# bharatlytics/faceRecognition_InfrenceEngine

Hardware: AMD Instinct MI355X
Metric: faces/sec end-to-end @1080p (higher is better)
Workload: dtype f16

## Files before the change

### facerecognition_infrenceengine_amd/csrc/ro_conv2.hip

```cpp
#include "detect_math.h"

namespace {

struct Rc2Args {
    const unsigned char* xs;
    const float* w;
    const float* bias; const float* slope;
    float* y;
    const int32_t* counts; int cap;
    int nslots, per_block;
    int32_t* zero;
};

template <int WIN, int HB, int WOUT, int HC, int G, int NCT, int NPH, int NBAND, int BROWS, int PR, int PO, int PROUNDS, int NBUFS, int DEPTH_>
struct Rc2Cfg {
    static constexpr int P = WIN + 2;
    static constexpr int NPX = G * HC * WOUT;
    static constexpr int NT = (NPX + 15) / 16;
    static constexpr int NTW = (NT + NPH - 1) / NPH;
    static constexpr int PLANE = G * HB * P * 64;
    static constexpr int NW = NCT * NPH;
    static constexpr int NPIECE = (2 * PLANE + 1023) / 1024;
    static constexpr int NPW = (NPIECE + NW - 1) / NW;
    static constexpr int COUT = NCT * 16;
    static constexpr int PC = COUT / PROUNDS;
    static constexpr int CS = PC + 4;
    static constexpr int POOL_BYTES = NPX * CS * 4;
    static constexpr int BUF = NPIECE * 1024 > POOL_BYTES ? NPIECE * 1024 : (POOL_BYTES + 1023) / 1024 * 1024;
    static constexpr int PRM_OFF = NBUFS * BUF;
    static constexpr int LDS_BYTES = PRM_OFF + 2 * COUT * 4;
    static constexpr int SLOT_BYTES = WIN * WIN * 128;
    static constexpr int KC = WOUT % 8, GK = (HC * WOUT) % 8;
    static constexpr int NTHR = NW * 64;
    static constexpr int NSTEP = 9 * NTW;
    static constexpr int DEPTH = DEPTH_;
    static constexpr int DMA_EVERY = (NSTEP * 5 / 8) / NPW > 0 ? (NSTEP * 5 / 8) / NPW : 1;
    static constexpr int Q4 = PC / 4;
    static_assert(NBUFS == 1 || NSTEP - 4 >= NPW, "every piece of the next item is issued inside the K loop");
    static_assert(NCT % PROUNDS == 0, "pool rounds");
    static_assert(2 * PLANE + 3 * P * 64 < 65536, "ds_read immediates");
    static_assert(2 * (PR - 1) + 2 < HC && 2 * (PO - 1) + 2 < WOUT + 0 * BROWS, "pool windows lie inside the band");
};

template <int WIN, int HB, int WOUT, int HC, int G, int NCT, int NPH, int NBAND, int BROWS, int PR, int PO, int PROUNDS, int NBUFS, int DEPTH_, int MINW>
__global__ __launch_bounds__(NCT * NPH * 64, MINW) void ro_conv2_split_kernel(Rc2Args a) {
#if defined(__HIP_DEVICE_COMPILE__)
    using C = Rc2Cfg<WIN, HB, WOUT, HC, G, NCT, NPH, NBAND, BROWS, PR, PO, PROUNDS, NBUFS, DEPTH_>;
    extern __shared__ __attribute__((aligned(16))) char lds2[];
    const int tid = threadIdx.x, lane = tid & 63, wave = tid >> 6;
    const int li = lane & 15, kq = lane >> 4;
    const int ct = wave % NCT, ph = wave / NCT;
    const int nitems = (a.nslots + G - 1) / G * NBAND;
    const int it_end = min(nitems, (int)(blockIdx.x + 1) * a.per_block);
    if (a.zero && blockIdx.x == 0 && tid == 0) *a.zero = 0;
    auto next_valid = [&](int it) {
        while (it < it_end) {
            const int s0 = it / NBAND * G;
            bool any = false;
            int last = s0;
#pragma unroll
            for (int g = 0; g < G; ++g) {
                const int sl = s0 + g;
                if (sl < a.nslots) {
                    const int f = sl / a.cap;
                    any = any || sl - f * a.cap < a.counts[f];
                    last = sl;
                }
            }
            if (any) return it;
            const int nxt = ((last / a.cap + 1) * a.cap) / G * NBAND;
            it = nxt > it ? nxt : it + 1;
        }
        return -1;
    };
    int cur = next_valid(blockIdx.x * a.per_block);
    if (cur < 0) return;

    half8 wh[9], wl[9];
    {
        const float* wrow = a.w + (size_t)(ct * 16 + li) * 9 * 32 + 8 * kq;
#pragma unroll
        for (int tap = 0; tap < 9; ++tap) {
            const float4v v0 = *reinterpret_cast<const float4v*>(wrow + tap * 32);
            const float4v v1 = *reinterpret_cast<const float4v*>(wrow + tap * 32 + 4);
#pragma unroll
            for (int j = 0; j < 8; ++j) {
                split_f16(j < 4 ? v0[j] : v1[j - 4], wh[tap], wl[tap], j);
            }
        }
    }
    const float4v bias_r = *reinterpret_cast<const float4v*>(a.bias + ct * 16 + 4 * kq);
    const float4v slope_r = *reinterpret_cast<const float4v*>(a.slope + ct * 16 + 4 * kq);
    bool mono = true;
    for (int c = 0; c < C::COUT; ++c) mono = mono && a.slope[c] >= 0.f;

    unsigned voff[C::NPW];
#pragma unroll
    for (int i = 0; i < C::NPW; ++i) {
        const int n = (wave + C::NW * i) * 64 + lane;
        unsigned o = 0x80000000u;
        if (n < 2 * C::PLANE / 16) {
            const int pl = n / (C::PLANE / 16), m = n - pl * (C::PLANE / 16);
            const int row = m >> 2, cp = m & 3;
            const int g = row / (HB * C::P), rr = row - g * (HB * C::P);
            const int Y = rr / C::P, X = rr - Y * C::P;
            if (X < WIN) {
                const int key = ((X + C::KC * Y + C::GK * g) >> 1) & 3;
                o = (unsigned)(g * C::SLOT_BYTES + (Y * WIN + X) * 128 + pl * 64 + ((cp ^ key) << 4));
            }
        }
        voff[i] = o;
    }
    auto item_rsrc = [&](int it) {
        const int sg = it / NBAND, band = it - sg * NBAND;
        const int s0 = sg * G;
        const unsigned char* base = a.xs + (size_t)s0 * C::SLOT_BYTES + (size_t)band * BROWS * WIN * 128;
        const int nsl = min(G, a.nslots - s0);
        const unsigned bytes = NBAND == 1 ? (unsigned)nsl * C::SLOT_BYTES : (unsigned)(HB * WIN * 128);
        return buffer_rsrc(base, bytes);
    };
    auto piece = [&](__amdgpu_buffer_rsrc_t rs, int buf, int i) {
        const int j = wave + C::NW * i;
        if (j < C::NPIECE)
            __builtin_amdgcn_raw_ptr_buffer_load_lds(rs, (lds_ptr_t)(lds2 + buf * C::BUF + j * 1024), 16, voff[i], 0, 0, 0);
    };
    const unsigned lbase = (unsigned)reinterpret_cast<uintptr_t>((lds_ptr_t)lds2);
    unsigned rt[C::NTW];
#pragma unroll
    for (int k = 0; k < C::NTW; ++k) {
        const int q = min((ph + k * NPH) * 16 + li, C::NPX - 1);
        const int g = q / (HC * WOUT), qq = q - g * (HC * WOUT);
        const int y = qq / WOUT, x = qq - y * WOUT;
        rt[k] = lbase + ((g * HB + y) * C::P + x) * 64;
    }

    float* prm = reinterpret_cast<float*>(lds2 + C::PRM_OFF);
    for (int c = tid; c < C::COUT; c += C::NTHR) { prm[c] = a.bias[c]; prm[C::COUT + c] = a.slope[c]; }
    if (NBUFS == 2) {
        const __amdgpu_buffer_rsrc_t rs0 = item_rsrc(cur);
#pragma unroll
        for (int i = 0; i < C::NPW; ++i) piece(rs0, 0, i);
    }
    int nxt = next_valid(cur + 1);
    for (int b = 0; cur >= 0; b ^= (NBUFS - 1)) {
        const int sg = cur / NBAND, band = cur - sg * NBAND;
        const int s0 = sg * G;
        unsigned smask = 0;
#pragma unroll
        for (int g = 0; g < G; ++g) {
            const int sl = s0 + g;
            if (sl < a.nslots) {
                const int f = sl / a.cap;
                if (sl - f * a.cap < a.counts[f]) smask |= 1u << g;
            }
        }
        if (NBUFS == 1) {
            __syncthreads();
            const __amdgpu_buffer_rsrc_t rs0 = item_rsrc(cur);
#pragma unroll
            for (int i = 0; i < C::NPW; ++i) piece(rs0, 0, i);
        }
        asm volatile("s_waitcnt vmcnt(0)" ::: "memory");
        __syncthreads();
        const __amdgpu_buffer_rsrc_t rsn = item_rsrc(nxt >= 0 ? nxt : cur);
        const int nn = nxt >= 0 ? next_valid(nxt + 1) : -1;

        float4v acc[C::NTW];
#pragma unroll
        for (int k = 0; k < C::NTW; ++k) acc[k] = float4v{0.f, 0.f, 0.f, 0.f};
        const unsigned boff = b ? (unsigned)C::BUF : 0u;
        unsigned xd[8];
#pragma unroll
        for (int d = 0; d < 8; ++d) xd[d] = boff + (unsigned)((kq ^ (((li + d) & 7) >> 1)) << 4);
        half8 fh[C::DEPTH + 1], fl[C::DEPTH + 1];
        auto rd = [&](auto S) {
            constexpr int s = decltype(S)::value;
            constexpr int tap = s / C::NTW, k = s - tap * C::NTW, kh = tap / 3, kw = tap - kh * 3;
            constexpr int imm = (kh * C::P + kw) * 64;
            unsigned ad;
            const unsigned r0 = rt[k], x0 = xd[(kw + C::KC * kh) & 7];
            half8& h = fh[s % (C::DEPTH + 1)];
            half8& l = fl[s % (C::DEPTH + 1)];
            asm volatile("v_add_u32 %2, %3, %4\n\tds_read_b128 %0, %2 offset:%5\n\tds_read_b128 %1, %2 offset:%6"
                         : "=&v"(h), "=&v"(l), "=&v"(ad)
                         : "v"(r0), "v"(x0), "n"(imm), "n"(imm + C::PLANE));
        };
        static_for<C::DEPTH>([&](auto S) { rd(S); });
        static_for<C::NSTEP>([&](auto S) {
            constexpr int s = decltype(S)::value;
            constexpr int tap = s / C::NTW, k = s - tap * C::NTW;
            if constexpr (s + C::DEPTH < C::NSTEP) rd(std::integral_constant<int, s + C::DEPTH>{});
            if constexpr (NBUFS == 2 && s >= 2 && (s - 2) % C::DMA_EVERY == 0 && (s - 2) / C::DMA_EVERY < C::NPW) {
                if (nxt >= 0) piece(rsn, b ^ 1, (s - 2) / C::DMA_EVERY);
            }
            constexpr int later = (C::NSTEP - 1 - s) < C::DEPTH ? (C::NSTEP - 1 - s) : C::DEPTH;
            half8& bh = fh[s % (C::DEPTH + 1)];
            half8& bl = fl[s % (C::DEPTH + 1)];
            asm volatile("s_waitcnt lgkmcnt(%2)" : "+v"(bh), "+v"(bl) : "n"(2 * later));
            acc[k] = __builtin_amdgcn_mfma_f32_16x16x32_f16(wh[tap], bh, acc[k], 0, 0, 0);
            acc[k] = __builtin_amdgcn_mfma_f32_16x16x32_f16(wl[tap], bh, acc[k], 0, 0, 0);
            acc[k] = __builtin_amdgcn_mfma_f32_16x16x32_f16(wh[tap], bl, acc[k], 0, 0, 0);
        });

        float* pt = reinterpret_cast<float*>(lds2 + b * C::BUF);
#pragma unroll
        for (int round = 0; round < PROUNDS; ++round) {
            __syncthreads();
            if (ct / (NCT / PROUNDS) == round) {
#pragma unroll
                for (int k = 0; k < C::NTW; ++k) {
                    const int q = (ph + k * NPH) * 16 + li;
                    if (q < C::NPX) {
                        float4v v = acc[k];
                        if (!mono) {
                            v += bias_r;
#pragma unroll
                            for (int e = 0; e < 4; ++e) v[e] = v[e] > 0.f ? v[e] : v[e] * slope_r[e];
                        }
                        *reinterpret_cast<float4v*>(pt + q * C::CS + (ct % (NCT / PROUNDS)) * 16 + 4 * kq) = v;
                    }
                }
            }
            __syncthreads();
            constexpr int Q4 = C::Q4;
            for (int e = tid; e < G * PR * PO * Q4; e += C::NTHR) {
                const int qd = e % Q4, pp = e / Q4;
                const int g = pp / (PR * PO), p2 = pp - g * (PR * PO);
                const int pr = p2 / PO, pc = p2 - pr * PO;
                const int slot = s0 + g;
                if (!((smask >> g) & 1)) continue;
                const float* src = pt + ((g * HC + 2 * pr) * WOUT + 2 * pc) * C::CS + qd * 4;
                float4v m = *reinterpret_cast<const float4v*>(src);
#pragma unroll
                for (int dy = 0; dy < 3; ++dy)
#pragma unroll
                    for (int dx = 0; dx < 3; ++dx) {
                        if (dy == 0 && dx == 0) continue;
                        const float4v v = *reinterpret_cast<const float4v*>(src + (dy * WOUT + dx) * C::CS);
#pragma unroll
                        for (int k = 0; k < 4; ++k) m[k] = fmaxf(m[k], v[k]);
                    }
                const int co = round * C::PC + qd * 4;
                if (mono) {
                    m += *reinterpret_cast<const float4v*>(prm + co);
                    const float4v sv = *reinterpret_cast<const float4v*>(prm + C::COUT + co);
#pragma unroll
                    for (int k = 0; k < 4; ++k) m[k] = m[k] > 0.f ? m[k] : m[k] * sv[k];
                }
                *reinterpret_cast<float4v*>(a.y + (((size_t)slot * PO + band * PR + pr) * PO + pc) * C::COUT + co) = m;
            }
        }
        cur = nxt; nxt = nn;
    }
#endif
}

template <int WIN, int HB, int WOUT, int HC, int G, int NCT, int NPH, int NBAND, int BROWS, int PR, int PO, int PROUNDS, int NBUFS, int DEPTH_, int MINW>
int launch_rc2(Rc2Args a, hipStream_t s) {
    using C = Rc2Cfg<WIN, HB, WOUT, HC, G, NCT, NPH, NBAND, BROWS, PR, PO, PROUNDS, NBUFS, DEPTH_>;
    auto kern = ro_conv2_split_kernel<WIN, HB, WOUT, HC, G, NCT, NPH, NBAND, BROWS, PR, PO, PROUNDS, NBUFS, DEPTH_, MINW>;
    const size_t lds = C::LDS_BYTES;
    if (lds > 64 * 1024) {
        static FrDevLatch latch;
        if (!fr_raise_lds(reinterpret_cast<const void*>(kern), lds, latch)) {
            fr_set_error("fr_ro_conv2_split: cannot raise dynamic LDS to %zu bytes", lds);
            return FR_E_LAUNCH;
        }
    }
    const int nitems = (a.nslots + G - 1) / G * NBAND;
    const int resident = 256 * (MINW * 4 / C::NW);
    int per = (nitems + 2 * resident - 1) / (2 * resident);
    if (per < 1) per = 1;
    a.per_block = per;
    kern<<<(nitems + per - 1) / per, C::NTHR, lds, s>>>(a);
    return FR_OK;
}

__global__ void ro_margin_list_kernel(const float* head, int nhead, const int32_t* counts, int nslots, int cap, float lthr,
                                      float margin, int32_t* list, int32_t* lcount, int lcap) {
    const int slot = blockIdx.x * 256 + threadIdx.x;
    if (slot >= nslots) return;
    const int f = slot / cap;
    if (slot - f * cap >= counts[f]) return;
    const float* h = head + (size_t)slot * nhead;
    const float d = h[1] - h[0];
    bool nonfinite = split_nonfinite(d);
    for (int i = 2; i < nhead; ++i) nonfinite = nonfinite || split_nonfinite(h[i]);
    if (nonfinite || fabsf(d - lthr) <= margin) {
        const int pos = atomicAdd(lcount, 1);
        if (pos < lcap) list[pos] = slot;
    }
}

__global__ void ro_scatter_rows_kernel(const float* src, const int32_t* list, const int32_t* lcount, int lcap, int ncols, float* dst) {
    const int n = min(*lcount, lcap);
    const int e = blockIdx.x * 256 + threadIdx.x;
    const int i = e / ncols, c = e - i * ncols;
    if (i < n) dst[(size_t)list[i] * ncols + c] = src[(size_t)i * ncols + c];
}

}

extern "C" int fr_ro_conv2_split(int net, const void* x_split, const float* w, const float* bias, const float* slope, float* y,
                                 int nslots, const int32_t* counts, int cap, int32_t* zero_word, fr_stream_t stream) {
    FR_REQUIRE(x_split && w && bias && slope && y && counts, "fr_ro_conv2_split: null pointer");
    FR_REQUIRE(nslots > 0 && cap > 0 && nslots % cap == 0, "fr_ro_conv2_split: nslots must be frames x cap");
    Rc2Args a{(const unsigned char*)x_split, w, bias, slope, y, counts, cap, nslots, 1, zero_word};
    hipStream_t s = fr_stream(stream);
    int rc;
    if (net == 0) rc = launch_rc2<11, 11, 9, 9, 3, 3, 4, 1, 0, 4, 4, 1, 2, 2, 3>(a, s);
    else if (net == 1) rc = launch_rc2<23, 13, 21, 11, 1, 4, 1, 2, 10, 5, 10, 1, 1, 3, 2>(a, s);
    else { FR_REQUIRE(false, "fr_ro_conv2_split: net must be 0 (R-Net) or 1 (O-Net)"); }
    if (rc != FR_OK) return rc;
    FR_CHECK_LAUNCH("ro_conv2_split_kernel");
    return FR_OK;
}

extern "C" int fr_ro_margin_list(const float* head, int nhead, const int32_t* counts, int nframes, int cap, float logit_thr,
                                 float margin, int32_t* list, int32_t* list_count, int list_cap, fr_stream_t stream) {
    FR_REQUIRE(head && counts && list && list_count, "fr_ro_margin_list: null pointer");
    FR_REQUIRE(nhead >= 2 && nframes > 0 && cap > 0 && list_cap > 0 && margin >= 0.f, "fr_ro_margin_list: bad argument");
    hipStream_t s = fr_stream(stream);
    const int nslots = nframes * cap;
    ro_margin_list_kernel<<<(nslots + 255) / 256, 256, 0, s>>>(head, nhead, counts, nslots, cap, logit_thr, margin, list, list_count, list_cap);
    FR_CHECK_LAUNCH("ro_margin_list_kernel");
    return FR_OK;
}

extern "C" int fr_ro_scatter_rows(const float* src, const int32_t* list, const int32_t* list_count, int list_cap, int ncols,
                                  float* dst, fr_stream_t stream) {
    FR_REQUIRE(src && list && list_count && dst && list_cap > 0 && ncols > 0, "fr_ro_scatter_rows: bad argument");
    ro_scatter_rows_kernel<<<(list_cap * ncols + 255) / 256, 256, 0, fr_stream(stream)>>>(src, list, list_count, list_cap, ncols, dst);
    FR_CHECK_LAUNCH("ro_scatter_rows_kernel");
    return FR_OK;
}
```

Baseline: 25360.

## Overlap R-Net conv2 max-pool of previous item with next item's MFMA loop

For the R-Net configuration, the conv2 kernel now writes each item's activations to a dedicated LDS tile. The 3x3 max-pool and store of that item is deferred into the next item's K loop, with groups of four waves taking turns at staggered steps, so pooling and global stores hide behind MFMA work. Slot-validity masks are now computed once in next_valid, which reads counts through scalar constant loads and is moved into the middle of the K loop. Max uses fmed3 against +inf. The extra LDS tile raises shared memory per block, which may cut occupancy, and the DMA issue schedule shifts later in the loop.

```diff
diff --git a/facerecognition_infrenceengine_amd/csrc/ro_conv2.hip b/facerecognition_infrenceengine_amd/csrc/ro_conv2.hip
--- a/facerecognition_infrenceengine_amd/csrc/ro_conv2.hip
+++ b/facerecognition_infrenceengine_amd/csrc/ro_conv2.hip
@@ -1,6 +1,17 @@
 #include "detect_math.h"
 
 namespace {
+
+__device__ __forceinline__ float opaque_inf() {
+    float r;
+    asm("v_mov_b32 %0, 0x7f800000" : "=v"(r));
+    return r;
+}
+__device__ __forceinline__ float vmax(float x, float y, float pinf) { return __builtin_amdgcn_fmed3f(x, y, pinf); }
+
+__device__ __forceinline__ int32_t ld_uniform(const int32_t* p, int i) {
+    return reinterpret_cast<const __attribute__((address_space(4))) int32_t*>(reinterpret_cast<uintptr_t>(p))[i];
+}
 
 struct Rc2Args {
     const unsigned char* xs;
@@ -12,7 +23,7 @@
     int32_t* zero;
 };
 
-template <int WIN, int HB, int WOUT, int HC, int G, int NCT, int NPH, int NBAND, int BROWS, int PR, int PO, int PROUNDS, int NBUFS, int DEPTH_>
+template <int WIN, int HB, int WOUT, int HC, int G, int NCT, int NPH, int NBAND, int BROWS, int PR, int PO, int PROUNDS, int NBUFS, int DEPTH_, bool OVL>
 struct Rc2Cfg {
     static constexpr int P = WIN + 2;
     static constexpr int NPX = G * HC * WOUT;
@@ -26,8 +37,11 @@
     static constexpr int PC = COUT / PROUNDS;
     static constexpr int CS = PC + 4;
     static constexpr int POOL_BYTES = NPX * CS * 4;
-    static constexpr int BUF = NPIECE * 1024 > POOL_BYTES ? NPIECE * 1024 : (POOL_BYTES + 1023) / 1024 * 1024;
-    static constexpr int PRM_OFF = NBUFS * BUF;
+    static constexpr int TCS = COUT + 4;
+    static constexpr int TILE_BYTES = NPX * TCS * 4;
+    static constexpr int BUF = OVL || NPIECE * 1024 > POOL_BYTES ? NPIECE * 1024 : (POOL_BYTES + 1023) / 1024 * 1024;
+    static constexpr int TILE_OFF = NBUFS * BUF;
+    static constexpr int PRM_OFF = TILE_OFF + (OVL ? TILE_BYTES : 0);
     static constexpr int LDS_BYTES = PRM_OFF + 2 * COUT * 4;
     static constexpr int SLOT_BYTES = WIN * WIN * 128;
     static constexpr int KC = WOUT % 8, GK = (HC * WOUT) % 8;
@@ -36,16 +50,21 @@
     static constexpr int DEPTH = DEPTH_;
     static constexpr int DMA_EVERY = (NSTEP * 5 / 8) / NPW > 0 ? (NSTEP * 5 / 8) / NPW : 1;
     static constexpr int Q4 = PC / 4;
+    static constexpr int PSLOTS = NW / 4;
+    static constexpr int PGAP = 2;
+    static constexpr int DMA0 = OVL ? 2 + (PSLOTS - 1) * PGAP : 2;
+    static_assert(!OVL || (NBUFS == 2 && PROUNDS == 1 && NW % 4 == 0), "overlapped pool");
+    static_assert(NBUFS == 1 || DMA0 + (NPW - 1) * DMA_EVERY <= NSTEP - 4, "the last piece is issued well inside the K loop");
     static_assert(NBUFS == 1 || NSTEP - 4 >= NPW, "every piece of the next item is issued inside the K loop");
     static_assert(NCT % PROUNDS == 0, "pool rounds");
     static_assert(2 * PLANE + 3 * P * 64 < 65536, "ds_read immediates");
     static_assert(2 * (PR - 1) + 2 < HC && 2 * (PO - 1) + 2 < WOUT + 0 * BROWS, "pool windows lie inside the band");
 };
 
-template <int WIN, int HB, int WOUT, int HC, int G, int NCT, int NPH, int NBAND, int BROWS, int PR, int PO, int PROUNDS, int NBUFS, int DEPTH_, int MINW>
+template <int WIN, int HB, int WOUT, int HC, int G, int NCT, int NPH, int NBAND, int BROWS, int PR, int PO, int PROUNDS, int NBUFS, int DEPTH_, int MINW, bool OVL>
 __global__ __launch_bounds__(NCT * NPH * 64, MINW) void ro_conv2_split_kernel(Rc2Args a) {
 #if defined(__HIP_DEVICE_COMPILE__)
-    using C = Rc2Cfg<WIN, HB, WOUT, HC, G, NCT, NPH, NBAND, BROWS, PR, PO, PROUNDS, NBUFS, DEPTH_>;
+    using C = Rc2Cfg<WIN, HB, WOUT, HC, G, NCT, NPH, NBAND, BROWS, PR, PO, PROUNDS, NBUFS, DEPTH_, OVL>;
     extern __shared__ __attribute__((aligned(16))) char lds2[];
     const int tid = threadIdx.x, lane = tid & 63, wave = tid >> 6;
     const int li = lane & 15, kq = lane >> 4;
@@ -53,27 +72,29 @@
     const int nitems = (a.nslots + G - 1) / G * NBAND;
     const int it_end = min(nitems, (int)(blockIdx.x + 1) * a.per_block);
     if (a.zero && blockIdx.x == 0 && tid == 0) *a.zero = 0;
-    auto next_valid = [&](int it) {
+    auto next_valid = [&](int it, unsigned& mask) {
         while (it < it_end) {
             const int s0 = it / NBAND * G;
-            bool any = false;
+            unsigned m = 0;
             int last = s0;
 #pragma unroll
             for (int g = 0; g < G; ++g) {
                 const int sl = s0 + g;
                 if (sl < a.nslots) {
                     const int f = sl / a.cap;
-                    any = any || sl - f * a.cap < a.counts[f];
+                    if (sl - f * a.cap < ld_uniform(a.counts, f)) m |= 1u << g;
                     last = sl;
                 }
             }
-            if (any) return it;
+            if (m) { mask = m; return it; }
             const int nxt = ((last / a.cap + 1) * a.cap) / G * NBAND;
             it = nxt > it ? nxt : it + 1;
         }
+        mask = 0;
         return -1;
     };
-    int cur = next_valid(blockIdx.x * a.per_block);
+    unsigned smask, nxt_mask;
+    int cur = next_valid(blockIdx.x * a.per_block, smask);
     if (cur < 0) return;
 
     half8 wh[9], wl[9];
@@ -134,6 +155,8 @@
         rt[k] = lbase + ((g * HB + y) * C::P + x) * 64;
     }
 
+    const float pinf = opaque_inf();
+
     float* prm = reinterpret_cast<float*>(lds2 + C::PRM_OFF);
     for (int c = tid; c < C::COUT; c += C::NTHR) { prm[c] = a.bias[c]; prm[C::COUT + c] = a.slope[c]; }
     if (NBUFS == 2) {
@@ -141,19 +164,42 @@
 #pragma unroll
         for (int i = 0; i < C::NPW; ++i) piece(rs0, 0, i);
     }
-    int nxt = next_valid(cur + 1);
-    for (int b = 0; cur >= 0; b ^= (NBUFS - 1)) {
+    auto pool_prev = [&](int s0p, int bandp, unsigned maskp) {
+        const float* pt = reinterpret_cast<const float*>(lds2 + C::TILE_OFF);
+        constexpr int Q4 = C::COUT / 4;
+        for (int e = tid; e < G * PR * PO * Q4; e += C::NTHR) {
+            const int qd = e % Q4, pp = e / Q4;
+            const int g = pp / (PR * PO), p2 = pp - g * (PR * PO);
+            const int pr = p2 / PO, pc = p2 - pr * PO;
+            if (!((maskp >> g) & 1)) continue;
+            const float* src = pt + ((g * HC + 2 * pr) * WOUT + 2 * pc) * C::TCS + qd * 4;
+            float4v m = *reinterpret_cast<const float4v*>(src);
+#pragma unroll
+            for (int dy = 0; dy < 3; ++dy)
+#pragma unroll
+                for (int dx = 0; dx < 3; ++dx) {
+                    if (dy == 0 && dx == 0) continue;
+                    const float4v v = *reinterpret_cast<const float4v*>(src + (dy * WOUT + dx) * C::TCS);
+#pragma unroll
+                    for (int k = 0; k < 4; ++k) m[k] = vmax(m[k], v[k], pinf);
+                }
+            const int co = qd * 4;
+            if (mono) {
+                m += *reinterpret_cast<const float4v*>(prm + co);
+                const float4v sv = *reinterpret_cast<const float4v*>(prm + C::COUT + co);
+#pragma unroll
+                for (int k = 0; k < 4; ++k) m[k] = m[k] > 0.f ? m[k] : m[k] * sv[k];
+            }
+            *reinterpret_cast<float4v*>(a.y + (((size_t)(s0p + g) * PO + bandp * PR + pr) * PO + pc) * C::COUT + co) = m;
+        }
+    };
+    int nxt = next_valid(cur + 1, nxt_mask);
+    int pv_s0 = 0, pv_band = 0;
+    unsigned pv_mask = 0;
+    int b = 0;
+    for (; cur >= 0; b ^= (NBUFS - 1)) {
         const int sg = cur / NBAND, band = cur - sg * NBAND;
         const int s0 = sg * G;
-        unsigned smask = 0;
-#pragma unroll
-        for (int g = 0; g < G; ++g) {
-            const int sl = s0 + g;
-            if (sl < a.nslots) {
-                const int f = sl / a.cap;
-                if (sl - f * a.cap < a.counts[f]) smask |= 1u << g;
-            }
-        }
         if (NBUFS == 1) {
             __syncthreads();
             const __amdgpu_buffer_rsrc_t rs0 = item_rsrc(cur);
@@ -163,7 +209,8 @@
         asm volatile("s_waitcnt vmcnt(0)" ::: "memory");
         __syncthreads();
         const __amdgpu_buffer_rsrc_t rsn = item_rsrc(nxt >= 0 ? nxt : cur);
-        const int nn = nxt >= 0 ? next_valid(nxt + 1) : -1;
+        int nn = -1;
+        unsigned nn_mask = 0;
 
         float4v acc[C::NTW];
 #pragma unroll
@@ -190,8 +237,14 @@
             constexpr int s = decltype(S)::value;
             constexpr int tap = s / C::NTW, k = s - tap * C::NTW;
             if constexpr (s + C::DEPTH < C::NSTEP) rd(std::integral_constant<int, s + C::DEPTH>{});
-            if constexpr (NBUFS == 2 && s >= 2 && (s - 2) % C::DMA_EVERY == 0 && (s - 2) / C::DMA_EVERY < C::NPW) {
-                if (nxt >= 0) piece(rsn, b ^ 1, (s - 2) / C::DMA_EVERY);
+            if constexpr (NBUFS == 2 && s >= C::DMA0 && (s - C::DMA0) % C::DMA_EVERY == 0 && (s - C::DMA0) / C::DMA_EVERY < C::NPW) {
+                if (nxt >= 0) piece(rsn, b ^ 1, (s - C::DMA0) / C::DMA_EVERY);
+            }
+            if constexpr (s == C::NSTEP / 2) {
+                if (nxt >= 0) nn = next_valid(nxt + 1, nn_mask);
+            }
+            if constexpr (OVL && s >= 1 && (s - 1) % C::PGAP == 0 && (s - 1) / C::PGAP < C::PSLOTS) {
+                if (pv_mask && (wave >> 2) == (s - 1) / C::PGAP) pool_prev(pv_s0, pv_band, pv_mask);
             }
             constexpr int later = (C::NSTEP - 1 - s) < C::DEPTH ? (C::NSTEP - 1 - s) : C::DEPTH;
             half8& bh = fh[s % (C::DEPTH + 1)];
@@ -202,6 +255,24 @@
             acc[k] = __builtin_amdgcn_mfma_f32_16x16x32_f16(wh[tap], bl, acc[k], 0, 0, 0);
         });
 
+        if constexpr (OVL) {
+            __syncthreads();
+            float* tw = reinterpret_cast<float*>(lds2 + C::TILE_OFF) + ct * 16 + 4 * kq;
+#pragma unroll
+            for (int k = 0; k < C::NTW; ++k) {
+                const int q = (ph + k * NPH) * 16 + li;
+                if (q < C::NPX) {
+                    float4v v = acc[k];
+                    if (!mono) {
+                        v += bias_r;
+#pragma unroll
+                        for (int e = 0; e < 4; ++e) v[e] = v[e] > 0.f ? v[e] : v[e] * slope_r[e];
+                    }
+                    *reinterpret_cast<float4v*>(tw + q * C::TCS) = v;
+                }
+            }
+            pv_s0 = s0; pv_band = band; pv_mask = smask;
+        } else {
         float* pt = reinterpret_cast<float*>(lds2 + b * C::BUF);
 #pragma unroll
         for (int round = 0; round < PROUNDS; ++round) {
@@ -250,15 +321,20 @@
                 *reinterpret_cast<float4v*>(a.y + (((size_t)slot * PO + band * PR + pr) * PO + pc) * C::COUT + co) = m;
             }
         }
-        cur = nxt; nxt = nn;
+        }
+        cur = nxt; smask = nxt_mask; nxt = nn; nxt_mask = nn_mask;
+    }
+    if constexpr (OVL) {
+        __syncthreads();
+        if (pv_mask) pool_prev(pv_s0, pv_band, pv_mask);
     }
 #endif
 }
 
-template <int WIN, int HB, int WOUT, int HC, int G, int NCT, int NPH, int NBAND, int BROWS, int PR, int PO, int PROUNDS, int NBUFS, int DEPTH_, int MINW>
+template <int WIN, int HB, int WOUT, int HC, int G, int NCT, int NPH, int NBAND, int BROWS, int PR, int PO, int PROUNDS, int NBUFS, int DEPTH_, int MINW, bool OVL>
 int launch_rc2(Rc2Args a, hipStream_t s) {
-    using C = Rc2Cfg<WIN, HB, WOUT, HC, G, NCT, NPH, NBAND, BROWS, PR, PO, PROUNDS, NBUFS, DEPTH_>;
-    auto kern = ro_conv2_split_kernel<WIN, HB, WOUT, HC, G, NCT, NPH, NBAND, BROWS, PR, PO, PROUNDS, NBUFS, DEPTH_, MINW>;
+    using C = Rc2Cfg<WIN, HB, WOUT, HC, G, NCT, NPH, NBAND, BROWS, PR, PO, PROUNDS, NBUFS, DEPTH_, OVL>;
+    auto kern = ro_conv2_split_kernel<WIN, HB, WOUT, HC, G, NCT, NPH, NBAND, BROWS, PR, PO, PROUNDS, NBUFS, DEPTH_, MINW, OVL>;
     const size_t lds = C::LDS_BYTES;
     if (lds > 64 * 1024) {
         static FrDevLatch latch;
@@ -308,8 +384,8 @@
     Rc2Args a{(const unsigned char*)x_split, w, bias, slope, y, counts, cap, nslots, 1, zero_word};
     hipStream_t s = fr_stream(stream);
     int rc;
-    if (net == 0) rc = launch_rc2<11, 11, 9, 9, 3, 3, 4, 1, 0, 4, 4, 1, 2, 2, 3>(a, s);
-    else if (net == 1) rc = launch_rc2<23, 13, 21, 11, 1, 4, 1, 2, 10, 5, 10, 1, 1, 3, 2>(a, s);
+    if (net == 0) rc = launch_rc2<11, 11, 9, 9, 3, 3, 4, 1, 0, 4, 4, 1, 2, 2, 3, true>(a, s);
+    else if (net == 1) rc = launch_rc2<23, 13, 21, 11, 1, 4, 1, 2, 10, 5, 10, 1, 1, 3, 2, false>(a, s);
     else { FR_REQUIRE(false, "fr_ro_conv2_split: net must be 0 (R-Net) or 1 (O-Net)"); }
     if (rc != FR_OK) return rc;
     FR_CHECK_LAUNCH("ro_conv2_split_kernel");
```

After: 25370 (median of 2 runs). About the same (+0.1%).
